# somanshu25/GPU-Accelerated-Point-Cloud-Registration-Using-Hierarchical-GMM

Measured on AMD Instinct MI355X. Metric: EM iterations/sec (N points x J components); E-step achieved HBM GB/s, higher is better.
Workload: dtype f32; 1 GPU; BASELINE configs[2]/[4]: uniform [0,1)^3 cloud, N=1,000,000 pts per GPU (seed=rank), flat diag GMM J=800 (flavour W), fused device-resident EM, tol=0; N>1: frames are shards of one joint fit, all-reduce of (7J+2) f64 sufficient statistics per iteration; points_per_gpu=1000000, components=800, cov_type=diag, device= (gfx950:sramecc+:xnack-), compute_units=256

## Files before the change

### gpu-accelerated-point-cloud-registration-using-hierarchical-gmm_amd/csrc/flat_kernels.hip

```cpp
#include "hgmm_ctx.h"
#include "wave_ops.h"

#include <type_traits>

#include <algorithm>
#include <cmath>
#include <cstdlib>
#include <cstring>

namespace hgmm {

constexpr float NEG_INF = -__builtin_huge_valf();
constexpr float LOG2E = 1.4426950408889634f;
constexpr float LN2 = 0.6931471805599453f;
constexpr int PK_MU = 0, PK_G = 3, PK_C = 6, PK_W = 7;
constexpr int PK_ROWS = 8;
typedef float f2 __attribute__((ext_vector_type(2)));
constexpr int WAVES_PER_BLOCK = 4;
constexpr int BLOCK = WAVES_PER_BLOCK * 64;

__device__ inline void pack_values(int j, bool valid, int Jpad, int variant, const float (&m)[3], const float (&i)[3],
                                   float wj, float* pack) {
    float m0 = 0.f, m1 = 0.f, m2 = 0.f, g0 = 0.f, g1 = 0.f, g2 = 0.f, c = NEG_INF;
    if (valid) {
// ... 499 lines not shown
                f2 a = cc[p] - (d0 * g0[p]) * d0;
                a = a - (d1 * g1[p]) * d1;
                a = a - (d2 * g2[p]) * d2;
                wl[r][p] = a;
            }
            wls[r] = NEG_INF;
            if (ODD) {
                const float d0 = x[r][0] - mu0s, d1 = x[r][1] - mu1s, d2 = x[r][2] - mu2s;
                float a = fmaf(-(d0 * g0s), d0, cs);
                a = fmaf(-(d1 * g1s), d1, a);
                a = fmaf(-(d2 * g2s), d2, a);
                wls[r] = a;
            }
        };
        auto store = [&](int r) {
            const int64_t row = g * ROWS + r;
            if (row < n) {
                float* out = log_prob + row * (int64_t)J;
#pragma unroll
                for (int v = 0; v < NV4; ++v) {
                    const int jb = (v * 64 + lane) * 4;
                    if (jb < J) store_f4<true>(out + jb, wl[r][2 * v].x, wl[r][2 * v].y, wl[r][2 * v + 1].x, wl[r][2 * v + 1].y);
                }
#pragma unroll
                for (int v = 0; v < NV1; ++v) {
                    const int j = 256 * NV4 + v * 64 + lane;
                    const int k = 4 * NV4 + v;
                    const float val = (ODD && k == K - 1) ? wls[r] : ((k & 1) ? wl[r][k >> 1].y : wl[r][k >> 1].x);
                    if (j < J) store_f1<true>(out + j, val);
                }
            }
        };
        if (LATE) {
#pragma unroll
            for (int r = 0; r < ROWS; ++r) compute(r);
            asm volatile("" ::: "memory");
            pacer.wait();
#pragma unroll
            for (int r = 0; r < ROWS; ++r) store(r);
        } else {
#pragma unroll
            for (int r = 0; r < ROWS; ++r) { compute(r); store(r); }
        }
#pragma unroll
        for (int r = 0; r < ROWS; ++r) { x[r][0] = nx[r][0]; x[r][1] = nx[r][1]; x[r][2] = nx[r][2]; }
    }
}

template <int NV4, int NV1>
__global__ __launch_bounds__(BLOCK) void flat_predict_rows_kernel(
    const float* __restrict__ X, const float* __restrict__ pack, int64_t n, int J, int Jpad,
    int32_t* __restrict__ labels) {
    using L = Layout<NV4, NV1>;
    constexpr int K = L::K;
    constexpr int KP = 2 * NV4 + NV1 / 2;
    constexpr bool ODD = (NV1 & 1) != 0;
    constexpr int ROWS = 4;
    const int lane = lane_id();
    f2 mu0[KP + 1], mu1[KP + 1], mu2[KP + 1], g0[KP + 1], g1[KP + 1], g2[KP + 1], cc[KP + 1];
    float mu0s = 0.f, mu1s = 0.f, mu2s = 0.f, g0s = 0.f, g1s = 0.f, g2s = 0.f, cs = NEG_INF;
    auto ld = [&](int row, int j) { return pack[row * Jpad + j]; };
#pragma unroll
    for (int p = 0; p < KP; ++p) {
        const int ja = L::j_of(2 * p, lane), jb = L::j_of(2 * p + 1, lane);
        mu0[p] = f2{ld(PK_MU + 0, ja), ld(PK_MU + 0, jb)};
        mu1[p] = f2{ld(PK_MU + 1, ja), ld(PK_MU + 1, jb)};
        mu2[p] = f2{ld(PK_MU + 2, ja), ld(PK_MU + 2, jb)};
        g0[p] = f2{ld(PK_G + 0, ja), ld(PK_G + 0, jb)};
        g1[p] = f2{ld(PK_G + 1, ja), ld(PK_G + 1, jb)};
        g2[p] = f2{ld(PK_G + 2, ja), ld(PK_G + 2, jb)};
        cc[p] = f2{ld(PK_C, ja), ld(PK_C, jb)};
    }
    if (ODD) {
        const int j = L::j_of(K - 1, lane);
        mu0s = ld(PK_MU + 0, j); mu1s = ld(PK_MU + 1, j); mu2s = ld(PK_MU + 2, j);
        g0s = ld(PK_G + 0, j); g1s = ld(PK_G + 1, j); g2s = ld(PK_G + 2, j);
        cs = ld(PK_C, j);
    }
    float njf[K];
#pragma unroll
    for (int k = 0; k < K; ++k) njf[k] = -(float)L::j_of(k, lane);

    const int64_t nw = (int64_t)gridDim.x * WAVES_PER_BLOCK;
    const int64_t gw = (int64_t)blockIdx.x * WAVES_PER_BLOCK + wave_in_block();
    const int64_t ngroups = (n + ROWS - 1) / ROWS;
    float x[ROWS][3];
    auto load_group = [&](int64_t g, float (&dst)[ROWS][3]) {
#pragma unroll
        for (int r = 0; r < ROWS; ++r) {
            int64_t row = g * ROWS + r;
            row = row < n ? row : n - 1;
            const float* xp = X + 3 * row;
            dst[r][0] = xp[0]; dst[r][1] = xp[1]; dst[r][2] = xp[2];
        }
    };
    if (gw < ngroups) load_group(gw, x);
    for (int64_t g = gw; g < ngroups; g += nw) {
        float nx[ROWS][3];
        load_group((g + nw < ngroups) ? g + nw : g, nx);
        f2 wl[ROWS][KP + 1];
        float wls[ROWS];
        float m[ROWS];
#pragma unroll
        for (int r = 0; r < ROWS; ++r) {
            const f2 X0 = f2{x[r][0], x[r][0]}, X1 = f2{x[r][1], x[r][1]}, X2 = f2{x[r][2], x[r][2]};
            float mm = NEG_INF;
#pragma unroll
            for (int p = 0; p < KP; ++p) {
                const f2 d0 = X0 - mu0[p], d1 = X1 - mu1[p], d2 = X2 - mu2[p];
                f2 a = cc[p] - (d0 * g0[p]) * d0;
                a = a - (d1 * g1[p]) * d1;
                a = a - (d2 * g2[p]) * d2;
                wl[r][p] = a;
                mm = fmaxf(mm, fmaxf(a.x, a.y));
            }
            wls[r] = NEG_INF;
            if (ODD) {
                const float d0 = x[r][0] - mu0s, d1 = x[r][1] - mu1s, d2 = x[r][2] - mu2s;
                float a = fmaf(-(d0 * g0s), d0, cs);
                a = fmaf(-(d1 * g1s), d1, a);
                a = fmaf(-(d2 * g2s), d2, a);
                wls[r] = a;
                mm = fmaxf(mm, a);
            }
            m[r] = mm;
        }
        wave_max4_dpp(m);
        float b[ROWS];
#pragma unroll
        for (int r = 0; r < ROWS; ++r) {
            float best = NEG_INF;
#pragma unroll
            for (int k = K - 1; k >= 0; --k) {
                const float val = (ODD && k == K - 1) ? wls[r] : ((k & 1) ? wl[r][k >> 1].y : wl[r][k >> 1].x);
                best = (val == m[r]) ? njf[k] : best;
            }
            b[r] = best;
        }
        wave_max4_dpp(b);
        if (lane < ROWS) {
            const int64_t row = g * ROWS + lane;
            const float mb = lane == 0 ? m[0] : lane == 1 ? m[1] : lane == 2 ? m[2] : m[3];
            const float bb = lane == 0 ? b[0] : lane == 1 ? b[1] : lane == 2 ? b[2] : b[3];
            int lab = (mb == NEG_INF || !(bb > NEG_INF)) ? 0 : (int)(-bb);
            if (lab >= J) lab = 0;
            if (row < n) labels[row] = lab;
        }
#pragma unroll
        for (int r = 0; r < ROWS; ++r) { x[r][0] = nx[r][0]; x[r][1] = nx[r][1]; x[r][2] = nx[r][2]; }
    }
}


template <int NSLOT>
__global__ __launch_bounds__(BLOCK) void flat_fused_pk_kernel(
    const float* __restrict__ X, const float* __restrict__ pack, int64_t n, int J, int Jpad,
    float* __restrict__ partials, double* __restrict__ lpn_partials,
    const int* __restrict__ done_flag, int allow_const_shift) {
    if (done_flag && *done_flag) return;
    constexpr int K = NSLOT;
    constexpr int KP = K / 2;
    constexpr bool ODD = (K & 1) != 0;
    const int lane = lane_id();
    f2 mu0[KP + 1], mu1[KP + 1], mu2[KP + 1], g0[KP + 1], g1[KP + 1], g2[KP + 1], cc[KP + 1];
    f2 s0[KP + 1], a0[KP + 1], a1[KP + 1], a2[KP + 1], b0[KP + 1], b1[KP + 1], b2[KP + 1];
    float mu0s = 0.f, mu1s = 0.f, mu2s = 0.f, g0s = 0.f, g1s = 0.f, g2s = 0.f, cs = NEG_INF;
    float s0s = 0.f, a0s = 0.f, a1s = 0.f, a2s = 0.f, b0s = 0.f, b1s = 0.f, b2s = 0.f;
#pragma unroll
    for (int p = 0; p < KP; ++p) {
        const int ja = (2 * p) * 64 + lane, jb = (2 * p + 1) * 64 + lane;
        mu0[p] = f2{pack[(PK_MU + 0) * Jpad + ja], pack[(PK_MU + 0) * Jpad + jb]};
        mu1[p] = f2{pack[(PK_MU + 1) * Jpad + ja], pack[(PK_MU + 1) * Jpad + jb]};
        mu2[p] = f2{pack[(PK_MU + 2) * Jpad + ja], pack[(PK_MU + 2) * Jpad + jb]};
        g0[p] = f2{pack[(PK_G + 0) * Jpad + ja], pack[(PK_G + 0) * Jpad + jb]};
        g1[p] = f2{pack[(PK_G + 1) * Jpad + ja], pack[(PK_G + 1) * Jpad + jb]};
        g2[p] = f2{pack[(PK_G + 2) * Jpad + ja], pack[(PK_G + 2) * Jpad + jb]};
        cc[p] = f2{pack[PK_C * Jpad + ja], pack[PK_C * Jpad + jb]};
        s0[p] = a0[p] = a1[p] = a2[p] = b0[p] = b1[p] = b2[p] = f2{0.f, 0.f};
    }
    if (ODD) {
        const int j = (K - 1) * 64 + lane;
        mu0s = pack[(PK_MU + 0) * Jpad + j]; mu1s = pack[(PK_MU + 1) * Jpad + j]; mu2s = pack[(PK_MU + 2) * Jpad + j];
        g0s = pack[(PK_G + 0) * Jpad + j]; g1s = pack[(PK_G + 1) * Jpad + j]; g2s = pack[(PK_G + 2) * Jpad + j];
        cs = pack[PK_C * Jpad + j];
    }

    float m0 = cs;
#pragma unroll
    for (int p = 0; p < KP; ++p) m0 = fmaxf(m0, fmaxf(cc[p].x, cc[p].y));
    m0 = wave_max_dpp(m0);
    const bool small_shift = allow_const_shift && m0 <= CS_MAX_SHIFT && m0 >= -64.0f;

    int64_t r0, r1;
    wave_row_range(n, r0, r1);
    double lsum = 0.0;
    float o0 = 0.f, o1 = 0.f, o2 = 0.f, ow = 0.f;
#pragma unroll
    for (int p = 0; p < KP; ++p) {
        const float wa = pack[PK_W * Jpad + (2 * p) * 64 + lane], wb = pack[PK_W * Jpad + (2 * p + 1) * 64 + lane];
        o0 = fmaf(wa, mu0[p].x, fmaf(wb, mu0[p].y, o0));
        o1 = fmaf(wa, mu1[p].x, fmaf(wb, mu1[p].y, o1));
        o2 = fmaf(wa, mu2[p].x, fmaf(wb, mu2[p].y, o2));
        ow += wa + wb;
    }
    if (ODD) {
        const float ws = pack[PK_W * Jpad + (K - 1) * 64 + lane];
        o0 = fmaf(ws, mu0s, o0); o1 = fmaf(ws, mu1s, o1); o2 = fmaf(ws, mu2s, o2);
        ow += ws;
    }
    {
        ow = wave_sum_dpp(ow);
        const float inv_w = ow > 0.f ? 1.0f / ow : 0.f;
        o0 = wave_sum_dpp(o0) * inv_w; o1 = wave_sum_dpp(o1) * inv_w; o2 = wave_sum_dpp(o2) * inv_w;
        if (!(fabsf(o0) < 3.0e38f)) o0 = 0.f;
        if (!(fabsf(o1) < 3.0e38f)) o1 = 0.f;
        if (!(fabsf(o2) < 3.0e38f)) o2 = 0.f;
    }
    auto rows = [&](auto cs_tag) {
    constexpr bool CS = decltype(cs_tag)::value;
    if (CS) {
        const f2 M0 = f2{m0, m0};
#pragma unroll
        for (int p = 0; p < KP; ++p) cc[p] = cc[p] - M0;
        cs -= m0;
    }
    const float eps_scale = __builtin_amdgcn_exp2f(-m0);
    float lacc = 0.f;
    float x0 = 0.f, x1 = 0.f, x2 = 0.f;
    if (r0 < r1) { const float* xp = X + 3 * r0; x0 = xp[0]; x1 = xp[1]; x2 = xp[2]; }
    for (int64_t row = r0; row < r1; ++row) {
        const int64_t nrow = (row + 1 < r1) ? row + 1 : row;
        const float* xn = X + 3 * nrow;
        const float nx0 = xn[0], nx1 = xn[1], nx2 = xn[2];
        const f2 X0 = f2{x0, x0}, X1 = f2{x1, x1}, X2 = f2{x2, x2};
        const float xo0 = x0 - o0, xo1 = x1 - o1, xo2 = x2 - o2;
        const f2 XO0 = f2{xo0, xo0}, XO1 = f2{xo1, xo1}, XO2 = f2{xo2, xo2};

        f2 wl[KP + 1];
        f2 q0[KP + 1], q1[KP + 1], q2[KP + 1];
        float q0s = 0.f, q1s = 0.f, q2s = 0.f;
        float wls = NEG_INF;
        float m = NEG_INF;
        f2 sacc = f2{0.f, 0.f};
#pragma unroll
        for (int p = 0; p < KP; ++p) {
            const f2 d0 = X0 - mu0[p], d1 = X1 - mu1[p], d2 = X2 - mu2[p];
            q0[p] = d0 * d0; q1[p] = d1 * d1; q2[p] = d2 * d2;
            f2 a = cc[p] - g0[p] * q0[p];
            a = a - g1[p] * q1[p];
            a = a - g2[p] * q2[p];
            if (CS) {
                wl[p] = f2{__builtin_amdgcn_exp2f(a.x), __builtin_amdgcn_exp2f(a.y)};
                sacc += wl[p];
            } else {
                wl[p] = a;
                m = fmaxf(m, fmaxf(a.x, a.y));
            }
        }
        if (ODD) {
            const float d0 = x0 - mu0s, d1 = x1 - mu1s, d2 = x2 - mu2s;
            q0s = d0 * d0; q1s = d1 * d1; q2s = d2 * d2;
            float a = fmaf(-g0s, q0s, cs);
            a = fmaf(-g1s, q1s, a);
            a = fmaf(-g2s, q2s, a);
            wls = CS ? __builtin_amdgcn_exp2f(a) : a;
            m = fmaxf(m, a);
        }
        if (CS) {
            m = m0;
        } else {
            m = wave_max_dpp(m);
            if (m == NEG_INF) m = 0.f;
            const f2 M = f2{m, m};
#pragma unroll
            for (int p = 0; p < KP; ++p) {
                const f2 t = wl[p] - M;
                wl[p] = f2{__builtin_amdgcn_exp2f(t.x), __builtin_amdgcn_exp2f(t.y)};
                sacc += wl[p];
            }
            if (ODD) wls = __builtin_amdgcn_exp2f(wls - m);
        }
        float s = sacc.x + sacc.y;
        if (ODD) s += wls;
        s = wave_sum_dpp(s);
        float inv_den;
        if (CS) {
            const float den = fmaf(FLAT_EPS, eps_scale, s);
            inv_den = __builtin_amdgcn_rcpf(den);
            lacc += __builtin_amdgcn_logf(den);
            if (((row - r0) & 7) == 7) {
                asm volatile("" ::: "memory");
                lsum += (double)lacc;
                lacc = 0.f;
            }
        } else {
            const float lpn2 = lpn2_from(m, s, inv_den);
            lsum += (double)(lpn2 * LN2);
        }
        const f2 INV = f2{inv_den, inv_den};
#pragma unroll
        for (int p = 0; p < KP; ++p) {
            const f2 rr = wl[p] * INV;
            s0[p] += rr;
            a0[p] += rr * XO0; a1[p] += rr * XO1; a2[p] += rr * XO2;
            b0[p] += rr * q0[p]; b1[p] += rr * q1[p]; b2[p] += rr * q2[p];
        }
        if (ODD) {
            const float rr = wls * inv_den;
            s0s += rr;
            a0s = fmaf(rr, xo0, a0s); a1s = fmaf(rr, xo1, a1s); a2s = fmaf(rr, xo2, a2s);
            b0s = fmaf(rr, q0s, b0s); b1s = fmaf(rr, q1s, b1s); b2s = fmaf(rr, q2s, b2s);
        }
        x0 = nx0; x1 = nx1; x2 = nx2;
    }
    if (CS) lsum = (lsum + (double)lacc + (double)(r1 > r0 ? r1 - r0 : 0) * (double)m0) * (double)LN2;
    };
    if (small_shift) rows(std::true_type{});
    else rows(std::false_type{});
    {
        const f2 O0 = f2{o0, o0}, O1 = f2{o1, o1}, O2 = f2{o2, o2};
#pragma unroll
        for (int p = 0; p < KP; ++p) {
            a0[p] -= (mu0[p] - O0) * s0[p]; a1[p] -= (mu1[p] - O1) * s0[p]; a2[p] -= (mu2[p] - O2) * s0[p];
        }
        if (ODD) {
            a0s = fmaf(-(mu0s - o0), s0s, a0s); a1s = fmaf(-(mu1s - o1), s0s, a1s); a2s = fmaf(-(mu2s - o2), s0s, a2s);
        }
    }

    __shared__ float sh[FLAT_NSTAT * NSLOT * 64];
    __shared__ double shl[WAVES_PER_BLOCK];
    const int w = wave_in_block();
    constexpr int ST = NSLOT * 64;
    if (lane == 0) shl[w] = lsum;
    auto put = [&](int k, bool first, float v0, float v1, float v2, float v3, float v4, float v5, float v6) {
        float* q = sh + k * 64 + lane;
        if (first) { q[0 * ST] = v0; q[1 * ST] = v1; q[2 * ST] = v2; q[3 * ST] = v3; q[4 * ST] = v4; q[5 * ST] = v5; q[6 * ST] = v6; }
        else { q[0 * ST] += v0; q[1 * ST] += v1; q[2 * ST] += v2; q[3 * ST] += v3; q[4 * ST] += v4; q[5 * ST] += v5; q[6 * ST] += v6; }
    };
    for (int turn = 0; turn < WAVES_PER_BLOCK; ++turn) {
        if (w == turn) {
#pragma unroll
            for (int p = 0; p < KP; ++p) {
                put(2 * p, turn == 0, s0[p].x, a0[p].x, a1[p].x, a2[p].x, b0[p].x, b1[p].x, b2[p].x);
                put(2 * p + 1, turn == 0, s0[p].y, a0[p].y, a1[p].y, a2[p].y, b0[p].y, b1[p].y, b2[p].y);
            }
            if (ODD) put(K - 1, turn == 0, s0s, a0s, a1s, a2s, b0s, b1s, b2s);
        }
        __syncthreads();
    }
    float* outp = partials + (size_t)blockIdx.x * FLAT_NSTAT * Jpad;
    for (int idx = threadIdx.x; idx < FLAT_NSTAT * ST; idx += BLOCK) {
        const int st = idx / ST, j = idx % ST;
        outp[st * Jpad + j] = sh[idx];
    }
    if (threadIdx.x == 0) {
        double t = 0.0;
        for (int i = 0; i < WAVES_PER_BLOCK; ++i) t += shl[i];
        lpn_partials[blockIdx.x] = t;
    }
}

template <int NV4, int NV1, bool ISLOG, bool NTLOAD>
__global__ __launch_bounds__(BLOCK) void flat_mstep_kernel(
    const float* __restrict__ X, const float* __restrict__ resp,
    const float* __restrict__ hint , int64_t n, int J, int Jpad,
    float* __restrict__ partials, int64_t ld, int round_robin) {
    using L = Layout<NV4, NV1>;
    constexpr int K = L::K;
    constexpr int KP = 2 * NV4 + NV1 / 2;
    constexpr bool ODD = (NV1 & 1) != 0;
    const int lane = lane_id();
    f2 c0[KP + 1], c1[KP + 1], c2[KP + 1];
    f2 s0[KP + 1], a0[KP + 1], a1[KP + 1], a2[KP + 1], b0[KP + 1], b1[KP + 1], b2[KP + 1];
    float c0s = 0.f, c1s = 0.f, c2s = 0.f, s0s = 0.f, a0s = 0.f, a1s = 0.f, a2s = 0.f, b0s = 0.f, b1s = 0.f, b2s = 0.f;
#pragma unroll
    for (int p = 0; p < KP; ++p) {
        const int ja = L::j_of(2 * p, lane), jb = L::j_of(2 * p + 1, lane);
        c0[p] = f2{hint[0 * Jpad + ja], hint[0 * Jpad + jb]};
        c1[p] = f2{hint[1 * Jpad + ja], hint[1 * Jpad + jb]};
        c2[p] = f2{hint[2 * Jpad + ja], hint[2 * Jpad + jb]};
        s0[p] = a0[p] = a1[p] = a2[p] = b0[p] = b1[p] = b2[p] = f2{0.f, 0.f};
    }
    if (ODD) {
        const int j = L::j_of(K - 1, lane);
        c0s = hint[0 * Jpad + j]; c1s = hint[1 * Jpad + j]; c2s = hint[2 * Jpad + j];
    }
    int64_t base, stride, cnt;
    {
        const int64_t nw = (int64_t)gridDim.x * WAVES_PER_BLOCK;
        const int64_t gw = (int64_t)blockIdx.x * WAVES_PER_BLOCK + wave_in_block();
        if (round_robin) {
            base = gw; stride = nw; cnt = (gw < n) ? (n - gw + nw - 1) / nw : 0;
        } else {
            int64_t r0, r1;
            wave_row_range(n, r0, r1);
            base = r0; stride = 1; cnt = r1 - r0;
        }
    }

    constexpr bool is_log = ISLOG;
    int off4[NV4 > 0 ? NV4 : 1], off1[NV1 > 0 ? NV1 : 1];
#pragma unroll
    for (int s = 0; s < NV4; ++s) { const int jb = (s * 64 + lane) * 4; off4[s] = (jb < J) ? jb : 0; }
#pragma unroll
    for (int s = 0; s < NV1; ++s) { const int j = 256 * NV4 + s * 64 + lane; off1[s] = (j < J) ? j : 0; }
    auto load_row = [&](int64_t row, float (&v)[K]) {
        const float* in = resp + row * ld;
#pragma unroll
        for (int s = 0; s < NV4; ++s) {
            typedef float f4v __attribute__((ext_vector_type(4)));
            const f4v* q = reinterpret_cast<const f4v*>(in + off4[s]);
            const f4v t = NTLOAD ? __builtin_nontemporal_load(q) : *q;
            v[s * 4 + 0] = t.x; v[s * 4 + 1] = t.y; v[s * 4 + 2] = t.z; v[s * 4 + 3] = t.w;
        }
#pragma unroll
        for (int s = 0; s < NV1; ++s) v[4 * NV4 + s] = NTLOAD ? __builtin_nontemporal_load(in + off1[s]) : in[off1[s]];
    };
    auto accumulate = [&](const float (&v)[K], float x0, float x1, float x2) {
        const f2 X0 = f2{x0, x0}, X1 = f2{x1, x1}, X2 = f2{x2, x2}, L2 = f2{LOG2E, LOG2E};
#pragma unroll
        for (int p = 0; p < KP; ++p) {
            f2 r = f2{v[2 * p], v[2 * p + 1]};
            if (is_log) {
                const f2 t = r * L2;
                r = f2{__builtin_amdgcn_exp2f(t.x), __builtin_amdgcn_exp2f(t.y)};
            }
            const f2 d0 = X0 - c0[p], d1 = X1 - c1[p], d2 = X2 - c2[p];
            const f2 rd0 = r * d0, rd1 = r * d1, rd2 = r * d2;
            s0[p] += r;
            a0[p] += rd0; a1[p] += rd1; a2[p] += rd2;
            b0[p] += rd0 * d0; b1[p] += rd1 * d1; b2[p] += rd2 * d2;
        }
        if (ODD) {
            const float r = is_log ? __builtin_amdgcn_exp2f(v[K - 1] * LOG2E) : v[K - 1];
            const float d0 = x0 - c0s, d1 = x1 - c1s, d2 = x2 - c2s;
            const float rd0 = r * d0, rd1 = r * d1, rd2 = r * d2;
            s0s += r;
            a0s += rd0; a1s += rd1; a2s += rd2;
            b0s = fmaf(rd0, d0, b0s); b1s = fmaf(rd1, d1, b1s); b2s = fmaf(rd2, d2, b2s);
        }
    };
    if (cnt > 0) {
        float bufa[K], bufb[K];
        load_row(base, bufa);
        const float* xp = X + 3 * base;
        float xa0 = xp[0], xa1 = xp[1], xa2 = xp[2];
        int64_t it = 0;
        for (; it + 2 <= cnt; it += 2) {
            const int64_t rb = base + (it + 1) * stride;
            __builtin_amdgcn_sched_barrier(0);
            load_row(rb, bufb);
            const float* xq = X + 3 * rb;
            const float xb0 = xq[0], xb1 = xq[1], xb2 = xq[2];
            __builtin_amdgcn_sched_barrier(0);
            accumulate(bufa, xa0, xa1, xa2);
            __builtin_amdgcn_sched_barrier(0);
            const int64_t ra = base + ((it + 2 < cnt) ? it + 2 : cnt - 1) * stride;
            load_row(ra, bufa);
            const float* xr = X + 3 * ra;
            xa0 = xr[0]; xa1 = xr[1]; xa2 = xr[2];
            __builtin_amdgcn_sched_barrier(0);
            accumulate(bufb, xb0, xb1, xb2);
            __builtin_amdgcn_sched_barrier(0);
        }
        if (it < cnt) accumulate(bufa, xa0, xa1, xa2);
    }
    __shared__ float sh[FLAT_NSTAT * L::CAP];
    const int w = wave_in_block();
    constexpr int ST = L::CAP;
    auto put = [&](int k, bool first, float v0, float v1, float v2, float v3, float v4, float v5, float v6) {
        float* q = sh + L::j_of(k, lane);
        if (L::j_of(k, lane) >= J) v0 = v1 = v2 = v3 = v4 = v5 = v6 = 0.f;
        if (first) { q[0 * ST] = v0; q[1 * ST] = v1; q[2 * ST] = v2; q[3 * ST] = v3; q[4 * ST] = v4; q[5 * ST] = v5; q[6 * ST] = v6; }
        else { q[0 * ST] += v0; q[1 * ST] += v1; q[2 * ST] += v2; q[3 * ST] += v3; q[4 * ST] += v4; q[5 * ST] += v5; q[6 * ST] += v6; }
    };
    for (int turn = 0; turn < WAVES_PER_BLOCK; ++turn) {
        if (w == turn) {
#pragma unroll
            for (int p = 0; p < KP; ++p) {
// ... 668 lines not shown
    else if (nv4 == 1 && nv1 == 2) ESTEP_R(1, 2);
    else if (nv4 == 0 && nv1 == 1) ESTEP_R(0, 1);
    else if (nv4 == 0 && nv1 == 2) ESTEP_R(0, 2);
    else return false;
#undef ESTEP_R
    return true;
}

static bool launch_logprob_rows(hgmm_ctx* c, int nv4, int nv1, float* log_prob) {
    const FlatState& f = c->flat;
    const bool have = (nv4 >= 1 && nv4 <= 3 && nv1 <= 2) || (nv4 == 4 && nv1 == 0) || (nv4 == 0 && (nv1 == 1 || nv1 == 2));
    if (!have) return false;
    const int64_t groups = (c->n + 3) / 4;
    const int64_t g64 = (int64_t)c->cus * 2;
    const int grid = (int)std::max<int64_t>(1, std::min<int64_t>(g64, (groups + WAVES_PER_BLOCK - 1) / WAVES_PER_BLOCK));
    const float* X = c->x_aos.as<float>();
    const float* pk = c->f_pack.as<float>();
    ProfScope prof(c, HGMM_K_FLAT_ESTEP);
    const int pace = store_pace16(c, grid, f.J, pace_target(c, f.J));
#define LOGP_R(A, B) flat_logprob_rows_pk_kernel<A, B, true><<<grid, BLOCK, 0, c->stream>>>(X, pk, c->n, f.J, f.Jpad, log_prob, pace)
    if (nv4 == 3 && nv1 == 1) LOGP_R(3, 1);
    else if (nv4 == 3 && nv1 == 0) LOGP_R(3, 0);
    else if (nv4 == 3 && nv1 == 2) LOGP_R(3, 2);
    else if (nv4 == 4 && nv1 == 0) LOGP_R(4, 0);
    else if (nv4 == 2 && nv1 == 0) LOGP_R(2, 0);
    else if (nv4 == 2 && nv1 == 1) LOGP_R(2, 1);
    else if (nv4 == 2 && nv1 == 2) LOGP_R(2, 2);
    else if (nv4 == 1 && nv1 == 0) LOGP_R(1, 0);
    else if (nv4 == 1 && nv1 == 1) LOGP_R(1, 1);
    else if (nv4 == 1 && nv1 == 2) LOGP_R(1, 2);
    else if (nv4 == 0 && nv1 == 1) LOGP_R(0, 1);
    else if (nv4 == 0 && nv1 == 2) LOGP_R(0, 2);
    else return false;
#undef LOGP_R
    return true;
}

static bool predict_rows_layout(const hgmm_ctx* c, int nv4, int nv1) {
    if (c->cfg[CFG_PREDICT_SINGLE_ROW]) return false;
    return (nv4 == 3 && nv1 <= 2) || (nv4 == 4 && nv1 == 0) || (nv4 == 2 && nv1 <= 2) || (nv4 == 1 && nv1 <= 2) ||
           (nv4 == 0 && (nv1 == 1 || nv1 == 2));
}
static bool launch_predict_rows(hgmm_ctx* c, int nv4, int nv1, int32_t* labels) {
    const FlatState& f = c->flat;
    const int grid = grid_for(c, (c->n + 3) / 4, c->n >= 400000 ? 8 : 4);
    const float* X = c->x_aos.as<float>();
    const float* pk = c->f_pack.as<float>();
#define PRED_R(A, B) flat_predict_rows_kernel<A, B><<<grid, BLOCK, 0, c->stream>>>(X, pk, c->n, f.J, f.Jpad, labels)
    if (nv4 == 3 && nv1 == 1) PRED_R(3, 1);
    else if (nv4 == 3 && nv1 == 0) PRED_R(3, 0);
    else if (nv4 == 3 && nv1 == 2) PRED_R(3, 2);
    else if (nv4 == 4 && nv1 == 0) PRED_R(4, 0);
    else if (nv4 == 2 && nv1 == 0) PRED_R(2, 0);
    else if (nv4 == 2 && nv1 == 1) PRED_R(2, 1);
    else if (nv4 == 2 && nv1 == 2) PRED_R(2, 2);
    else if (nv4 == 1 && nv1 == 0) PRED_R(1, 0);
    else if (nv4 == 1 && nv1 == 1) PRED_R(1, 1);
    else if (nv4 == 1 && nv1 == 2) PRED_R(1, 2);
    else if (nv4 == 0 && nv1 == 1) PRED_R(0, 1);
    else if (nv4 == 0 && nv1 == 2) PRED_R(0, 2);
    else return false;
#undef PRED_R
    return true;
}

static int estep_rows_grid(hgmm_ctx* c, bool cshift) {
    const bool after_mstep = c->flat.last_kernel == 2 || (c->flat.last_kernel == 1 && !c->flat.idle_since_launch);
    const int full = grid_for(c, (c->n + 3) / 4, after_mstep ? 2 : 1);
    if (after_mstep) return full;
    return cshift ? std::min(full, std::max(1, c->cus * 3 / 4)) : full;
}

template <bool NORMALISE>
static int launch_estep(hgmm_ctx* c, float* log_resp, float* lpn, int32_t* argmax, int* grid_out) {
    const FlatState& f = c->flat;
    const int grid = grid_for(c, c->n, 2);
    *grid_out = grid;
    const float* X = c->x_aos.as<float>();
    const float* pk = c->f_pack.as<float>();
    double* lp = c->f_lpn_partials.as<double>();
    int nv4, nv1;
    pick_layout(f.J, &nv4, &nv1);
    const bool nt = NORMALISE && f.J % 4 == 0;
    const int rr = 0;
    if (!NORMALISE && !log_resp && !lpn && argmax && predict_rows_layout(c, nv4, nv1)) {
        ProfScope prof(c, HGMM_K_FLAT_ESTEP);
        (void)launch_predict_rows(c, nv4, nv1, argmax);
        HGMM_HIP(c, hipGetLastError());
        return HGMM_OK;
    }
    if (!NORMALISE && log_resp && !lpn && !argmax) {
        if (launch_logprob_rows(c, nv4, nv1, log_resp)) {
            c->flat.last_kernel = 1;
            c->flat.idle_since_launch = false;
            HGMM_HIP(c, hipGetLastError());
            return HGMM_OK;
        }
    }
    const int rows = (NORMALISE && log_resp) ? 4 : 1;
    if (rows > 1) {
        const bool cshift = !argmax;
        const double target = pace_target(c, f.J);
        const int bpc_rows = (c->n >= 400000 && f.J <= 128) ? 4 : 2;
        const int grid_r = target > 0.0 ? grid_for(c, (c->n + 3) / 4, bpc_rows)
                                        : estep_rows_grid(c, cshift);
        const int pace = store_pace16(c, grid_r, f.J, target);
        c->flat.last_kernel = 1;
        c->flat.idle_since_launch = false;
        unsigned long long* stamp = nullptr;
        const bool observed = cshift && pace_observe_begin(c, target, 4.0 * (double)c->n * (double)f.J, grid_r, &stamp);
        bool launched;
        {
            ProfScope prof(c, HGMM_K_FLAT_ESTEP);
            launched = launch_estep_rows(c, nv4, nv1, grid_r, cshift, log_resp, lpn, argmax, pace, observed ? stamp : nullptr);
        }
        if (launched) {
            if (observed) pace_observe_end(c);
            *grid_out = grid_r;
            HGMM_HIP(c, hipGetLastError());
            return HGMM_OK;
        }
    }
    ProfScope prof(c, HGMM_K_FLAT_ESTEP);
#define ESTEP_M(A, B)                                                                              \
    do {                                                                                           \
        if (nt) flat_estep_kernel<A, B, NORMALISE, NORMALISE><<<grid, BLOCK, 0, c->stream>>>(       \
                    X, pk, c->n, f.J, f.Jpad, log_resp, lpn, argmax, lp, rr);                       \
        else flat_estep_kernel<A, B, NORMALISE, false><<<grid, BLOCK, 0, c->stream>>>(              \
                    X, pk, c->n, f.J, f.Jpad, log_resp, lpn, argmax, lp, rr);                       \
    } while (0)
    LAYOUT_DISPATCH(nv4, nv1, ESTEP_M);
#undef ESTEP_M
    HGMM_HIP(c, hipGetLastError());
    return HGMM_OK;
}

static int launch_fused(hgmm_ctx* c, const int* done_flag, int* grid_out, int* valid_j) {
    c->flat.last_kernel = 3;
    const FlatState& f = c->flat;
    if (!done_flag) done_flag = c->f_ctl.as<int>() + 16;
    const int ns = (f.J + 63) / 64;
    int grid;
    {
        const int bpc_max = ns <= 4 ? 8 : (ns <= 8 ? 6 : 4);
        const int64_t by_rows = c->n / (WAVES_PER_BLOCK * 100);
        const int64_t big = std::min<int64_t>(by_rows, std::min<int64_t>((int64_t)c->cus * bpc_max, FLAT_MAX_BLOCKS));
        grid = (int)std::max<int64_t>(grid_for(c, c->n, 2), big);
    }
    *grid_out = grid;
    const float* X = c->x_aos.as<float>();
    const float* pk = c->f_pack.as<float>();
    float* part = c->f_partials.as<float>();
    double* lp = c->f_lpn_partials.as<double>();
#define FUSED_CASE(S)                                                                           \
    do {                                                                                        \
        flat_fused_pk_kernel<S><<<grid, BLOCK, 0, c->stream>>>(X, pk, c->n, f.J, f.Jpad, part,  \
                                                              lp, done_flag, 1);              \
        *valid_j = S * 64;                                                                      \
    } while (0)
    ProfScope prof(c, HGMM_K_FLAT_FUSED);
    switch (ns) {
        case 1: FUSED_CASE(1); break;
        case 2: FUSED_CASE(2); break;
        case 3: FUSED_CASE(3); break;
        case 4: FUSED_CASE(4); break;
        case 5: FUSED_CASE(5); break;
        case 6: FUSED_CASE(6); break;
        case 7: FUSED_CASE(7); break;
        case 8: FUSED_CASE(8); break;
        case 9: FUSED_CASE(9); break;
        case 10: FUSED_CASE(10); break;
        case 11: FUSED_CASE(11); break;
        case 12: FUSED_CASE(12); break;
        case 13: FUSED_CASE(13); break;
        case 14: FUSED_CASE(14); break;
        case 15: FUSED_CASE(15); break;
        default: FUSED_CASE(16); break;
    }
#undef FUSED_CASE
    HGMM_HIP(c, hipGetLastError());
    return HGMM_OK;
}

static int launch_reduce(hgmm_ctx* c, int nblocks, int valid_j, bool with_lpn, const int* done_flag,
                         int n_lpn_blocks = -1) {
    const FlatState& f = c->flat;
    const int total = FLAT_NSTAT * f.Jpad;
    if (c->comm_on() || !done_flag) done_flag = c->f_ctl.as<int>() + 16;
    flat_reduce_kernel<<<(total + RED_IDX - 1) / RED_IDX + 1, RED_IDX * RED_SLICES, 0, c->stream>>>(
        c->f_partials.as<float>(), with_lpn ? c->f_lpn_partials.as<double>() : nullptr, nblocks,
        n_lpn_blocks < 0 ? nblocks : n_lpn_blocks, valid_j, f.Jpad, (double)c->n, c->f_stats.as<double>(),
        done_flag);
    HGMM_HIP(c, hipGetLastError());
    if (c->comm_on()) HGMM_TRY(allreduce_f64_dev(c, c->f_stats.as<double>(), (size_t)total + 2));
    return HGMM_OK;
}

static int chunk_valid(const FlatState& f, int ci) {
    const int rem = f.J - ci * CH_J;
    return rem < CH_J ? rem : CH_J;
}

static int chunk_normalisers(hgmm_ctx* c, bool want_arg, float* lpn_out, int32_t* argmax_out,
                             bool want_partials, int* n_lpn_blocks) {
    const FlatState& f = c->flat;
    const int grid = grid_for(c, c->n, 3);
    float* cm = c->f_cm.as<float>();
    float* cs = c->f_cs.as<float>();
    int* ca = c->f_ca.as<int>();
    for (int ci = 0; ci < f.nchunks; ++ci)
        flat_chunk_lse_kernel<<<grid, BLOCK, 0, c->stream>>>(
            c->x_aos.as<float>(), c->f_pack.as<float>() + ci * CH_J, c->n, chunk_valid(f, ci), ci * CH_J, f.Jpad,
            cm + (size_t)ci * c->n, cs + (size_t)ci * c->n, want_arg ? ca + (size_t)ci * c->n : nullptr);
    const int cblocks = (int)((c->n + 255) / 256);
    flat_chunk_combine_kernel<<<cblocks, 256, 0, c->stream>>>(cm, cs, want_arg ? ca : nullptr, f.nchunks, c->n,
                                                            c->f_lpn2.as<float>(), lpn_out, argmax_out,
                                                            want_partials ? c->f_lpn_partials.as<double>() : nullptr);
    HGMM_HIP(c, hipGetLastError());
    if (n_lpn_blocks) *n_lpn_blocks = cblocks;
    return HGMM_OK;
}

static int chunk_statistics(hgmm_ctx* c, const int* done_flag, int* grid_out) {
    const FlatState& f = c->flat;
    const int grid = grid_for(c, c->n, 2);
    {
        ProfScope prof(c, HGMM_K_FLAT_FUSED);
        for (int ci = 0; ci < f.nchunks; ++ci)
            flat_chunk_fused_kernel<<<grid, BLOCK, 0, c->stream>>>(
                c->x_aos.as<float>(), c->f_pack.as<float>() + ci * CH_J, c->n, f.Jpad, c->f_lpn2.as<float>(),
                c->f_partials.as<float>() + ci * CH_J, done_flag);
    }
    HGMM_HIP(c, hipGetLastError());
    *grid_out = grid;
    return HGMM_OK;
}

static int enqueue_em_iteration(hgmm_ctx* c) {
    FlatState& f = c->flat;
    int* ctl = c->f_ctl.as<int>();
    float* ctl_f = reinterpret_cast<float*>(ctl + 8);
    int grid = 0, valid_j = 0;
    if (f.chunked) {
        int n_lpn = 0;
        HGMM_TRY(chunk_normalisers(c, false, nullptr, nullptr, true, &n_lpn));
        HGMM_TRY(chunk_statistics(c, ctl, &grid));
        HGMM_TRY(launch_reduce(c, grid, f.nchunks * CH_J, true, ctl, n_lpn));
        flat_finalize_mb_kernel<<<(f.Jpad + 255) / 256, 256, 0, c->stream>>>(
            c->f_stats.as<double>(), c->f_pack.as<float>() + PK_MU * f.Jpad, f.J, f.Jpad, f.cov_type, f.variant,
            c->f_mu.as<float>(), c->f_cov.as<float>(), c->f_w.as<float>(), c->f_inv.as<float>(),
            c->f_pack.as<float>(), ctl);
        flat_ctl_kernel<<<1, 1, 0, c->stream>>>(c->f_stats.as<double>(), f.Jpad, c->f_lls.as<float>(), f.lls_cap,
                                               f.tol, ctl, ctl_f);
        HGMM_HIP(c, hipGetLastError());
        f.launched++;
        return HGMM_OK;
    }
    int* stop = ctl + ((f.launched & 1) ? 3 : 0);
    int* stop_next = ctl + ((f.launched & 1) ? 0 : 3);
    HGMM_TRY(launch_fused(c, stop, &grid, &valid_j));
    HGMM_TRY(launch_reduce(c, grid, valid_j, true, stop));
    flat_finalize_kernel<<<f.Jpad / 256, 256, 0, c->stream>>>(
        c->f_stats.as<double>(), c->f_pack.as<float>() + PK_MU * f.Jpad, f.J, f.Jpad, f.cov_type,
        f.variant, c->f_mu.as<float>(), c->f_cov.as<float>(), c->f_w.as<float>(), c->f_inv.as<float>(),
        c->f_pack.as<float>(), c->f_lls.as<float>(), f.lls_cap, f.tol, ctl, ctl_f, stop, stop_next);
    HGMM_HIP(c, hipGetLastError());
    f.launched++;
    return HGMM_OK;
}

}

using namespace hgmm;

__global__ __launch_bounds__(256) void flat_mean_lpn_kernel(const double* __restrict__ partials, int nblocks, double n,
                                                            double* __restrict__ out) {
    __shared__ double sh[4];
    double acc = 0.0;
    for (int i = threadIdx.x; i < nblocks; i += 256) acc += partials[i];
    acc = wave_sum_f64(acc);
    if (lane_id() == 0) sh[wave_in_block()] = acc;
    __syncthreads();
    if (threadIdx.x == 0) *out = (sh[0] + sh[1] + sh[2] + sh[3]) / n;
}

static int flat_estep_enqueue(hgmm_ctx* c, int cov_type, int variant, int J, const float* mu, const float* inv_std,
                              const float* w, float* dev_log_resp, float* dev_lpn, int32_t* dev_argmax, int* grid_out,
                              bool params_on_device = false) {
    HGMM_TRY(flat_check(c, cov_type, variant, J));
    HGMM_TRY(flat_setup(c, cov_type, variant, J));
    if (params_on_device) {
        if (!mu || !inv_std || !w) return fail(c, HGMM_ERR_ARG, "device parameter array is NULL");
        const FlatState& f = c->flat;
        flat_pack_kernel<<<(f.Jpad + 255) / 256, 256, 0, c->stream>>>(f.J, f.Jpad, f.cov_type, f.variant, mu, inv_std, w,
                                                                    c->f_pack.as<float>());
    } else {
        HGMM_TRY(flat_upload(c, mu, inv_std, false, w));
        launch_pack(c);
    }
    int grid = 0;
    if (c->flat.chunked) {
        const FlatState& f = c->flat;
        ProfScope prof(c, HGMM_K_FLAT_ESTEP);
        HGMM_TRY(chunk_normalisers(c, dev_argmax != nullptr, dev_lpn, dev_argmax, true, &grid));
        if (dev_log_resp) {
            const int g2 = grid_for(c, c->n, 2);
            for (int ci = 0; ci < f.nchunks; ++ci)
                flat_chunk_write_kernel<<<g2, BLOCK, 0, c->stream>>>(
                    c->x_aos.as<float>(), c->f_pack.as<float>() + ci * CH_J, c->n, chunk_valid(f, ci), f.Jpad,
                    c->f_lpn2.as<float>(), dev_log_resp + ci * CH_J, (int64_t)J);
// ... 407 lines not shown
```

Before: 2981 EM it/s (1M-pt x 800-comp frames x iterations per second, all GPUs).

## Pack half-filled tail slot so two rows share one wave's trailing lanes

When J leaves a trailing 64-wide slot with at most 32 valid components (J=800 gives 13 slots, the last holding 32), the fused E-step kernel now computes the tail for two consecutive rows in one pass. The low 32 lanes handle the current row and the high 32 lanes the next row, using exec-masked inline asm for the diffs, adds and multiplies. Half-lane partial statistics are folded together at the end with a shuffle. The aim is to halve the wasted exp/FMA work on the mostly-empty tail slot, at the cost of fragile inline asm, wave-uniform row bounds, and extra branching.

```diff
diff --git a/gpu-accelerated-point-cloud-registration-using-hierarchical-gmm_amd/csrc/flat_kernels.hip b/gpu-accelerated-point-cloud-registration-using-hierarchical-gmm_amd/csrc/flat_kernels.hip
--- a/gpu-accelerated-point-cloud-registration-using-hierarchical-gmm_amd/csrc/flat_kernels.hip
+++ b/gpu-accelerated-point-cloud-registration-using-hierarchical-gmm_amd/csrc/flat_kernels.hip
@@ -675,7 +675,33 @@
 }
 
 
-template <int NSLOT>
+struct TailWhole { static constexpr bool half = false; };
+struct TailHalf { static constexpr bool half = true; };
+constexpr uint64_t LANES_LO = 0x00000000ffffffffull, LANES_HI = 0xffffffff00000000ull;
+
+__device__ __forceinline__ void lanes_add(float& acc, float v, uint64_t mask) {
+    uint64_t saved;
+    asm volatile("s_nop 0\n\ts_and_saveexec_b64 %1, %3\n\tv_add_f32 %0, %0, %2\n\ts_mov_b64 exec, %1"
+                 : "+v"(acc), "=&s"(saved) : "v"(v), "s"(mask) : "scc");
+}
+__device__ __forceinline__ void lanes_mul(float& acc, float v, uint64_t mask) {
+    uint64_t saved;
+    asm volatile("s_nop 0\n\ts_and_saveexec_b64 %1, %3\n\tv_mul_f32 %0, %0, %2\n\ts_mov_b64 exec, %1"
+                 : "+v"(acc), "=&s"(saved) : "v"(v), "s"(mask) : "scc");
+}
+__device__ __forceinline__ void lanes_zero(float& acc, uint64_t mask) {
+    uint64_t saved;
+    asm volatile("s_and_saveexec_b64 %1, %2\n\tv_mov_b32 %0, 0\n\ts_mov_b64 exec, %1"
+                 : "+v"(acc), "=&s"(saved) : "s"(mask) : "scc");
+}
+__device__ __forceinline__ void lanes_diff(f2& d01, float& d2, f2 x01, float x2, f2 mu01, float mu2, uint64_t mask) {
+    uint64_t saved;
+    asm volatile("s_and_saveexec_b64 %2, %7\n\tv_pk_add_f32 %0, %3, %4 neg_lo:[0,1] neg_hi:[0,1]\n\t"
+                 "v_sub_f32 %1, %5, %6\n\ts_mov_b64 exec, %2"
+                 : "+v"(d01), "+v"(d2), "=&s"(saved) : "s"(x01), "v"(mu01), "s"(x2), "v"(mu2), "s"(mask) : "scc");
+}
+
+template <int NSLOT, class TAIL>
 __global__ __launch_bounds__(BLOCK) void flat_fused_pk_kernel(
     const float* __restrict__ X, const float* __restrict__ pack, int64_t n, int J, int Jpad,
     float* __restrict__ partials, double* __restrict__ lpn_partials,
@@ -684,6 +710,8 @@
     constexpr int K = NSLOT;
     constexpr int KP = K / 2;
     constexpr bool ODD = (K & 1) != 0;
+    constexpr bool HT = TAIL::half;
+    static_assert(ODD || !HT, "a half tail is the half-filled trailing single slot");
     const int lane = lane_id();
     f2 mu0[KP + 1], mu1[KP + 1], mu2[KP + 1], g0[KP + 1], g1[KP + 1], g2[KP + 1], cc[KP + 1];
     f2 s0[KP + 1], a0[KP + 1], a1[KP + 1], a2[KP + 1], b0[KP + 1], b1[KP + 1], b2[KP + 1];
@@ -701,12 +729,12 @@
         cc[p] = f2{pack[PK_C * Jpad + ja], pack[PK_C * Jpad + jb]};
         s0[p] = a0[p] = a1[p] = a2[p] = b0[p] = b1[p] = b2[p] = f2{0.f, 0.f};
     }
-    if (ODD) {
-        const int j = (K - 1) * 64 + lane;
+    auto load_single = [&](int j) {
         mu0s = pack[(PK_MU + 0) * Jpad + j]; mu1s = pack[(PK_MU + 1) * Jpad + j]; mu2s = pack[(PK_MU + 2) * Jpad + j];
         g0s = pack[(PK_G + 0) * Jpad + j]; g1s = pack[(PK_G + 1) * Jpad + j]; g2s = pack[(PK_G + 2) * Jpad + j];
         cs = pack[PK_C * Jpad + j];
-    }
+    };
+    if (ODD) load_single((K - 1) * 64 + (HT ? (lane & 31) : lane));
 
     float m0 = cs;
 #pragma unroll
@@ -716,6 +744,15 @@
 
     int64_t r0, r1;
     wave_row_range(n, r0, r1);
+    if (HT) {
+        auto uniform = [](int64_t v) {
+            const uint32_t lo = __builtin_amdgcn_readfirstlane((int)(uint32_t)(uint64_t)v);
+            const uint32_t hi = __builtin_amdgcn_readfirstlane((int)(uint32_t)((uint64_t)v >> 32));
+            return (int64_t)(((uint64_t)hi << 32) | lo);
+        };
+        r0 = uniform(r0); r1 = uniform(r1);
+    }
+    auto before_end = [&](int64_t row) { return HT ? row != r1 : row < r1; };
     double lsum = 0.0;
     float o0 = 0.f, o1 = 0.f, o2 = 0.f, ow = 0.f;
 #pragma unroll
@@ -727,7 +764,7 @@
         ow += wa + wb;
     }
     if (ODD) {
-        const float ws = pack[PK_W * Jpad + (K - 1) * 64 + lane];
+        const float ws = (HT && lane >= 32) ? 0.f : pack[PK_W * Jpad + (K - 1) * 64 + (HT ? (lane & 31) : lane)];
         o0 = fmaf(ws, mu0s, o0); o1 = fmaf(ws, mu1s, o1); o2 = fmaf(ws, mu2s, o2);
         ow += ws;
     }
@@ -741,6 +778,8 @@
     }
     auto rows = [&](auto cs_tag) {
     constexpr bool CS = decltype(cs_tag)::value;
+    constexpr bool SHARE = HT && CS;
+    if (HT && !CS) load_single((K - 1) * 64 + lane);
     if (CS) {
         const f2 M0 = f2{m0, m0};
 #pragma unroll
@@ -751,10 +790,14 @@
     float lacc = 0.f;
     float x0 = 0.f, x1 = 0.f, x2 = 0.f;
     if (r0 < r1) { const float* xp = X + 3 * r0; x0 = xp[0]; x1 = xp[1]; x2 = xp[2]; }
-    for (int64_t row = r0; row < r1; ++row) {
-        const int64_t nrow = (row + 1 < r1) ? row + 1 : row;
+    float td0 = 0.f, td1 = 0.f, td2 = 0.f, tw = 0.f;
+    for (int64_t row = r0; before_end(row); ++row) {
+        const int64_t nrow = before_end(row + 1) ? row + 1 : row;
         const float* xn = X + 3 * nrow;
         const float nx0 = xn[0], nx1 = xn[1], nx2 = xn[2];
+        const int odd = SHARE ? (int)(row - r0) & 1 : 1;
+        const int left = (int)(r1 - row);
+        const uint64_t owner = LANES_LO << (32 * odd);
         const f2 X0 = f2{x0, x0}, X1 = f2{x1, x1}, X2 = f2{x2, x2};
         const float xo0 = x0 - o0, xo1 = x1 - o1, xo2 = x2 - o2;
         const f2 XO0 = f2{xo0, xo0}, XO1 = f2{xo1, xo1}, XO2 = f2{xo2, xo2};
@@ -780,7 +823,21 @@
                 m = fmaxf(m, fmaxf(a.x, a.y));
             }
         }
-        if (ODD) {
+        if (SHARE) {
+            asm volatile("" : "+v"(sacc));
+            if (odd == 0) {
+                asm volatile("" ::: "memory");
+                const f2 MU01 = f2{mu0s, mu1s};
+                f2 d01 = f2{x0, x1} - MU01;
+                td2 = x2 - mu2s;
+                lanes_diff(d01, td2, f2{nx0, nx1}, nx2, MU01, mu2s, LANES_HI);
+                td0 = d01.x; td1 = d01.y;
+                float a = fmaf(-g0s, td0 * td0, cs);
+                a = fmaf(-g1s, td1 * td1, a);
+                a = fmaf(-g2s, td2 * td2, a);
+                tw = __builtin_amdgcn_exp2f(a);
+            }
+        } else if (ODD) {
             const float d0 = x0 - mu0s, d1 = x1 - mu1s, d2 = x2 - mu2s;
             q0s = d0 * d0; q1s = d1 * d1; q2s = d2 * d2;
             float a = fmaf(-g0s, q0s, cs);
@@ -804,7 +861,8 @@
             if (ODD) wls = __builtin_amdgcn_exp2f(wls - m);
         }
         float s = sacc.x + sacc.y;
-        if (ODD) s += wls;
+        if (SHARE) lanes_add(s, tw, owner);
+        else if (ODD) s += wls;
         s = wave_sum_dpp(s);
         float inv_den;
         if (CS) {
@@ -828,7 +886,16 @@
             a0[p] += rr * XO0; a1[p] += rr * XO1; a2[p] += rr * XO2;
             b0[p] += rr * q0[p]; b1[p] += rr * q1[p]; b2[p] += rr * q2[p];
         }
-        if (ODD) {
+        if (SHARE) {
+            lanes_mul(tw, inv_den, owner);
+            if ((1 - odd) * (left - 1) == 0) {
+                asm volatile("" ::: "memory");
+                if (odd != 1) lanes_zero(tw, LANES_HI);
+                s0s += tw;
+                a0s = fmaf(tw, td0, a0s); a1s = fmaf(tw, td1, a1s); a2s = fmaf(tw, td2, a2s);
+                b0s = fmaf(tw, td0 * td0, b0s); b1s = fmaf(tw, td1 * td1, b1s); b2s = fmaf(tw, td2 * td2, b2s);
+            }
+        } else if (ODD) {
             const float rr = wls * inv_den;
             s0s += rr;
             a0s = fmaf(rr, xo0, a0s); a1s = fmaf(rr, xo1, a1s); a2s = fmaf(rr, xo2, a2s);
@@ -846,9 +913,16 @@
         for (int p = 0; p < KP; ++p) {
             a0[p] -= (mu0[p] - O0) * s0[p]; a1[p] -= (mu1[p] - O1) * s0[p]; a2[p] -= (mu2[p] - O2) * s0[p];
         }
-        if (ODD) {
+        if (ODD && !(HT && small_shift)) {
             a0s = fmaf(-(mu0s - o0), s0s, a0s); a1s = fmaf(-(mu1s - o1), s0s, a1s); a2s = fmaf(-(mu2s - o2), s0s, a2s);
         }
+    }
+    if (HT && small_shift) {
+        auto fold = [&](float& v) {
+            const float up = __shfl_down(v, 32, 64);
+            v = lane < 32 ? v + up : 0.f;
+        };
+        fold(s0s); fold(a0s); fold(a1s); fold(a2s); fold(b0s); fold(b1s); fold(b2s);
     }
 
     __shared__ float sh[FLAT_NSTAT * NSLOT * 64];
@@ -1823,10 +1897,15 @@
     const float* pk = c->f_pack.as<float>();
     float* part = c->f_partials.as<float>();
     double* lp = c->f_lpn_partials.as<double>();
+    const bool half_tail = (ns & 1) && f.J - 64 * (ns - 1) <= 32;
 #define FUSED_CASE(S)                                                                           \
     do {                                                                                        \
-        flat_fused_pk_kernel<S><<<grid, BLOCK, 0, c->stream>>>(X, pk, c->n, f.J, f.Jpad, part,  \
-                                                              lp, done_flag, 1);              \
+        if (((S) & 1) && half_tail)                                                             \
+            flat_fused_pk_kernel<S, std::conditional<(S) & 1, TailHalf, TailWhole>::type>       \
+                <<<grid, BLOCK, 0, c->stream>>>(X, pk, c->n, f.J, f.Jpad, part, lp, done_flag, 1); \
+        else                                                                                    \
+            flat_fused_pk_kernel<S, TailWhole><<<grid, BLOCK, 0, c->stream>>>(X, pk, c->n, f.J, f.Jpad, part,  \
+                                                                         lp, done_flag, 1);     \
         *valid_j = S * 64;                                                                      \
     } while (0)
     ProfScope prof(c, HGMM_K_FLAT_FUSED);
```

Result: slower. 2852 EM it/s (1M-pt x 800-comp frames x iterations per second, all GPUs) (-4.3%).
